# alessioGalatolo/GAN-2D-to-3D

Hardware: AMD Instinct MI355X
Metric: GAN2Shape step iters/sec, faces 128×128 b=8, 1/2/4/8 MI355X (higher is better)
Workload: dtype f32; 1 GPU; face128_n8; image_size=128, gan_size=128, n_proj_samples=8, mfma_operands=f32, prior=ellipsoid, step_mix=7:7:6 (step1:step2:step3, main.py:148 stage 0), images_per_rank=1

## Files before the change

gan-2d-to-3d_amd/csrc/fused_bias_act.hip:

```cpp
#include "g2s_common.h"
#include <hip/hip_fp16.h>

namespace g2s {

enum { MODE_LIN = 0, MODE_ZERO = 1, MODE_LRELU = 2, MODE_LRELU_GRAD = 3 };

__device__ __forceinline__ float act_apply(int mode, float x, float ref, float alpha, float scale) {
    float y;
    switch (mode) {
    case MODE_ZERO: y = 0.0f; break;
    case MODE_LRELU: y = (x > 0.0f) ? x : x * alpha; break;
    case MODE_LRELU_GRAD: y = (ref > 0.0f) ? x : x * alpha; break;
    default: y = x; break;
    }
    return y * scale;
}

template <int MODE, bool BIAS>
__global__ __launch_bounds__(256) void fba_f32_vec4(const float4 *__restrict__ x,
                                                    const float *__restrict__ b,
                                                    const float4 *__restrict__ ref,
                                                    float4 *__restrict__ y, unsigned n4,
                                                    unsigned step_b4, unsigned size_b, float alpha,
                                                    float scale) {
// ... 166 lines not shown
        noise_bias_act_scalar<<<dim3(std::min(cdiv(HW, 256), 64), B * C), 256, 0, st>>>(
            x, noise, noise_w, bias, y, C, HW, alpha, scale);
    }
    return check_launch("g2s_noise_bias_act");
}

namespace g2s {

__global__ __launch_bounds__(256) void add_bias_scale_kernel(const float *a, const float *b, const float *bias,
                                                             float *y, int64_t n, int64_t hw, int C, float scale) {
    const bool vec = (n & 3) == 0 && (hw & 3) == 0 &&
                     ((reinterpret_cast<uintptr_t>(a) | reinterpret_cast<uintptr_t>(y) | reinterpret_cast<uintptr_t>(b)) & 15) == 0;
    const int64_t stride = (int64_t)gridDim.x * blockDim.x * 4;
    for (int64_t i = ((int64_t)blockIdx.x * blockDim.x + threadIdx.x) * 4; i < n; i += stride) {
        if (vec) {
            float4 v = *reinterpret_cast<const float4 *>(a + i);
            if (b) {
                const float4 w = *reinterpret_cast<const float4 *>(b + i);
                v.x += w.x;
                v.y += w.y;
                v.z += w.z;
                v.w += w.w;
            }
            const float bi = bias ? bias[(i / hw) % C] : 0.0f;
            *reinterpret_cast<float4 *>(y + i) = float4{(v.x + bi) * scale, (v.y + bi) * scale, (v.z + bi) * scale,
                                                        (v.w + bi) * scale};
        } else {
            for (int64_t j = i; j < i + 4 && j < n; j++)
                y[j] = (a[j] + (b ? b[j] : 0.0f) + (bias ? bias[(j / hw) % C] : 0.0f)) * scale;
        }
    }
}

__global__ void clamp_kernel(const float *__restrict__ x, const float *__restrict__ g, float *__restrict__ y,
                             int64_t n, float lo, float hi, int dir) {
    const int64_t stride = (int64_t)gridDim.x * blockDim.x * 4;
    for (int64_t i = ((int64_t)blockIdx.x * blockDim.x + threadIdx.x) * 4; i < n; i += stride) {
        if (i + 4 <= n && (((uintptr_t)(x + i) | (uintptr_t)(y + i) | (uintptr_t)(dir ? g + i : x + i)) & 15) == 0) {
            const float4 v = *reinterpret_cast<const float4 *>(x + i);
            float4 o;
            if (dir) {
                const float4 q = *reinterpret_cast<const float4 *>(g + i);
                o = float4{(v.x >= lo && v.x <= hi) ? q.x : 0.0f, (v.y >= lo && v.y <= hi) ? q.y : 0.0f,
                           (v.z >= lo && v.z <= hi) ? q.z : 0.0f, (v.w >= lo && v.w <= hi) ? q.w : 0.0f};
            } else {
                auto cl = [&](float t) { return t < lo ? lo : (t > hi ? hi : t); };
                o = float4{cl(v.x), cl(v.y), cl(v.z), cl(v.w)};
            }
            *reinterpret_cast<float4 *>(y + i) = o;
        } else {
            for (int64_t j = i; j < i + 4 && j < n; j++)
                y[j] = dir ? ((x[j] >= lo && x[j] <= hi) ? g[j] : 0.0f) : (x[j] < lo ? lo : (x[j] > hi ? hi : x[j]));
        }
    }
}

}

extern "C" int g2s_clamp(const float *x, const float *g, float *y, int64_t n, float lo, float hi, int backward,
                         g2s_stream_t stream) {
    G2S_REQUIRE(x && y && n > 0 && (!backward || g) && lo <= hi, "bad argument");
    const int64_t quads = (n + 3) / 4;
    const int blocks = (int)std::min<int64_t>((quads + 255) / 256, 256 * 8);
    g2s::clamp_kernel<<<blocks, 256, 0, g2s::as_stream(stream)>>>(x, g, y, n, lo, hi, backward ? 1 : 0);
    return g2s::check_launch("g2s_clamp");
}

extern "C" int g2s_add_bias_scale(const float *a, const float *b, const float *bias, float *y, int64_t n, int64_t hw,
                                  int C, float scale, g2s_stream_t stream) {
    G2S_REQUIRE(a && y, "a and y must not be NULL");
    G2S_REQUIRE(n > 0 && hw > 0 && C > 0, "n, hw, C must be positive");
    const int64_t quads = (n + 3) / 4;
    const int blocks = (int)std::min<int64_t>((quads + 255) / 256, 256 * 8);
    g2s::add_bias_scale_kernel<<<blocks, 256, 0, g2s::as_stream(stream)>>>(a, b, bias, y, n, hw, C, scale);
    return g2s::check_launch("g2s_add_bias_scale");
}
```

gan-2d-to-3d_amd/csrc/rowops.hip:

```cpp
#include <algorithm>
#include "g2s_common.h"
#include "wave_sum.h"

namespace g2s {

__global__ __launch_bounds__(256) void rows_dot_scale(const float *__restrict__ a,
                                                      const float *__restrict__ b,
                                                      const float *__restrict__ s,
                                                      const float *__restrict__ inv,
                                                      float *__restrict__ out,
                                                      float *__restrict__ dot, int rows, int n,
                                                      int aligned_bases) {
    const int row = blockIdx.x * 4 + (threadIdx.x >> 6), lane = threadIdx.x & 63;
    if (row >= rows) return;
    const size_t off = (size_t)row * n;
    const float *ar = a ? a + off : nullptr;
    const float *br = b + off;
    float *orow = out ? out + off : nullptr;
    const float sc = s ? s[row] : 1.0f;
    float acc = 0.0f;
    int head = aligned_bases ? (int)((4 - (off & 3)) & 3) : n;
    if (head > n) head = n;
    const int n4 = (n - head) >> 2, tail0 = head + 4 * n4;
    for (int i = lane; i < head; i += 64) {
// ... 39 lines not shown
    __shared__ float red[4][64];
    const int lane = threadIdx.x & 63, wave = threadIdx.x >> 6;
    float acc = 0.0f;
    if (i < Cin) {
#pragma unroll 8
        for (int o = wave; o < Cout; o += 4) {
            const float d = demod[b * Cout + o];
            acc += gd[b * Cout + o] * d * d * d * wsq[(size_t)o * Cin + i];
        }
    }
    red[wave][lane] = acc;
    __syncthreads();
    if (wave == 0 && i < Cin) {
        const float g = -s[b * Cin + i] * (red[0][lane] + red[1][lane] + red[2][lane] + red[3][lane]);
        store(b * Cin + i, g);
    }
}

__global__ __launch_bounds__(256) void demod_fwd(const float *__restrict__ wsq, const float *__restrict__ s,
                                                 float *__restrict__ demod, int B, int Cin, int Cout, float eps) {
    const int idx = blockIdx.x * 4 + (threadIdx.x >> 6);
    if (idx >= B * Cout) return;
    demod_fwd_one(wsq, s, demod, idx, threadIdx.x & 63, Cin, Cout, eps);
}

__global__ __launch_bounds__(256) void demod_bwd(const float *__restrict__ wsq, const float *__restrict__ s,
                                                 const float *__restrict__ demod, const float *__restrict__ gd,
                                                 const float *gs_add,
                                                 float *gs, int B, int Cin, int Cout) {
    demod_bwd_one(wsq, s, demod, gd, blockIdx.x * 64 + (threadIdx.x & 63), blockIdx.y, Cin, Cout,
                  [=](int at, float g) { gs[at] = gs_add ? gs_add[at] + g : g; });
}

__global__ __launch_bounds__(256) void synth_rows(const float *__restrict__ x, const float *__restrict__ g1,
                                                  const float *__restrict__ s1, const float *__restrict__ g2,
                                                  const float *__restrict__ s2, const float *__restrict__ noise,
                                                  const float *__restrict__ noise_w, const float *__restrict__ bias,
                                                  const float *__restrict__ demod, float *__restrict__ out,
                                                  float *__restrict__ dot1, float *__restrict__ dot2,
                                                  float *__restrict__ gdot, int rows, int channels, int n,
                                                  int noise_stride, float slope, float gain, int vec) {
    const int row = blockIdx.x * 4 + (threadIdx.x >> 6), lane = threadIdx.x & 63;
    if (row >= rows) return;
    const size_t off = (size_t)row * n;
    const float *xr = x + off, *g1r = g1 + off, *g2r = g2 ? g2 + off : nullptr;
    float *orow = out ? out + off : nullptr;
    const float a1 = s1[row], a2 = g2 ? s2[row] : 0.0f;
    float nw = 0.0f, bi = 0.0f;
    if (gdot) {
        const int b = row / channels;
        nw = noise_w[0];
        bi = bias[row - b * channels];
        noise += (size_t)b * noise_stride;
    }
    const float inv_gain = 1.0f / gain, inv_slope = 1.0f / slope;
    float d1 = 0.0f, d2 = 0.0f, dg = 0.0f;
    auto one = [&](float xv, float gv1, float gv2, float nz) {
        d1 += xv * gv1;
        d2 += xv * gv2;
        const float o = (gv1 * a1 + gv2 * a2) * (xv > 0.0f ? gain : gain * slope);
        if (gdot) dg += o * ((xv > 0.0f ? xv : xv * inv_slope) * inv_gain - nw * nz - bi);
        return o;
    };
    if (vec) {
        for (int i = lane; i < (n >> 2); i += 64) {
            const float4 xv = reinterpret_cast<const float4 *>(xr)[i];
            const float4 v1 = reinterpret_cast<const float4 *>(g1r)[i];
            const float4 v2 = g2r ? reinterpret_cast<const float4 *>(g2r)[i] : float4{0.f, 0.f, 0.f, 0.f};
            const float4 nz = gdot ? reinterpret_cast<const float4 *>(noise)[i] : float4{0.f, 0.f, 0.f, 0.f};
            float4 o;
            o.x = one(xv.x, v1.x, v2.x, nz.x);
            o.y = one(xv.y, v1.y, v2.y, nz.y);
            o.z = one(xv.z, v1.z, v2.z, nz.z);
            o.w = one(xv.w, v1.w, v2.w, nz.w);
            if (orow) reinterpret_cast<float4 *>(orow)[i] = o;
        }
    } else {
        for (int i = lane; i < n; i += 64) {
            const float o = one(xr[i], g1r[i], g2r ? g2r[i] : 0.0f, gdot ? noise[i] : 0.0f);
            if (orow) orow[i] = o;
        }
    }
    d1 = wave_sum(d1);
    d2 = wave_sum(d2);
    dg = wave_sum(dg);
    if (lane == 0) {
        dot1[row] = d1;
        if (dot2) dot2[row] = d2;
        if (gdot) gdot[row] = dg / demod[row];
    }
}

__global__ __launch_bounds__(256) void channel_sum(const float *__restrict__ g, float *__restrict__ out, int B, int C,
                                                   int n) {
    __shared__ float red[4];
    const int c = blockIdx.x, lane = threadIdx.x & 63, wave = threadIdx.x >> 6;
    float acc = 0.0f;
    const int total = B * n;
    for (int i = threadIdx.x; i < total; i += 256) acc += g[((size_t)(i / n) * C + c) * n + i % n];
    acc = wave_sum(acc);
    if (lane == 0) red[wave] = acc;
    __syncthreads();
    if (threadIdx.x == 0) out[c] = red[0] + red[1] + red[2] + red[3];
}

struct DemodMulti {
    const float *wsq[G2S_DEMOD_MAX_LAYERS], *s[G2S_DEMOD_MAX_LAYERS], *gd[G2S_DEMOD_MAX_LAYERS];
    float *demod[G2S_DEMOD_MAX_LAYERS], *gs[G2S_DEMOD_MAX_LAYERS];
    int Cin[G2S_DEMOD_MAX_LAYERS], Cout[G2S_DEMOD_MAX_LAYERS];
    int layers, B;
    float eps;
};

__global__ __launch_bounds__(256) void demod_fwd_multi(DemodMulti d) {
    const int l = blockIdx.y;
    const int idx = blockIdx.x * 4 + (threadIdx.x >> 6);
    if (idx >= d.B * d.Cout[l]) return;
    demod_fwd_one(d.wsq[l], d.s[l], d.demod[l], idx, threadIdx.x & 63, d.Cin[l], d.Cout[l], d.eps);
}

// ... 44 lines not shown

extern "C" int g2s_demod_bwd_multi(const void *const *wsq, const void *const *s, const void *const *demod,
                                   const void *const *gd, const void *const *gs, const int *Cin, const int *Cout,
                                   int layers, int B, g2s_stream_t stream) {
    G2S_REQUIRE(gd && gs, "gd, gs must not be NULL");
    DemodMulti d{};
    int mi, mo;
    const int rc = demod_multi_fill(d, wsq, s, demod, gd, gs, Cin, Cout, layers, B, mi, mo);
    if (rc != G2S_OK) return rc;
    for (int l = 0; l < layers; l++) G2S_REQUIRE(gd[l] && gs[l], "layer %d: gd / gs NULL", l);
    demod_bwd_multi<<<dim3(cdiv(mi, 64), B, layers), 256, 0, as_stream(stream)>>>(d);
    return check_launch("g2s_demod_bwd_multi");
}

extern "C" int g2s_channel_sum(const float *g, float *out, int B, int C, int n, g2s_stream_t stream) {
    G2S_REQUIRE(g && out && B > 0 && C > 0 && n > 0 && (long)B * n < (1l << 31), "bad argument");
    channel_sum<<<C, 256, 0, as_stream(stream)>>>(g, out, B, C, n);
    return check_launch("g2s_channel_sum");
}

static int synth_bwd_rows_launch(const char *who, int noise_stride, const float *x, const float *g1, const float *s1,
                                 const float *g2, const float *s2, const float *noise, const float *noise_w,
                                 const float *bias, const float *demod, float *out, float *dot1, float *dot2,
                                 float *gdot, int rows, int channels, int n, float slope, float gain,
                                 g2s_stream_t stream) {
    G2S_REQUIRE(x && g1 && s1 && dot1 && rows > 0 && channels > 0 && n > 0, "x, g1, s1, dot1 must not be NULL; sizes positive");
    G2S_REQUIRE((g2 == nullptr) == (s2 == nullptr) && (g2 == nullptr) == (dot2 == nullptr), "g2, s2, dot2 come together");
    G2S_REQUIRE(!gdot || (noise && noise_w && bias && demod), "gdot needs noise, noise_w, bias, demod");
    G2S_REQUIRE(slope > 0.0f && gain > 0.0f, "slope and gain must be positive (the activation is inverted)");
    uintptr_t bits = (uintptr_t)x | (uintptr_t)g1 | (uintptr_t)g2 | (uintptr_t)out | (gdot ? (uintptr_t)noise : 0);
    const int vec = (n % 4 == 0) && (bits & 15) == 0;
    if (noise_stride)
        G2S_REQUIRE(rows % channels == 0, "rows must be a multiple of channels with one noise map per sample");
    synth_rows<<<cdiv(rows, 4), 256, 0, as_stream(stream)>>>(x, g1, s1, g2, s2, noise, noise_w, bias, demod, out, dot1,
                                                               dot2, gdot, rows, channels, n, noise_stride, slope, gain,
                                                               vec);
    return check_launch(who);
}

extern "C" int g2s_synth_bwd_rows(const float *x, const float *g1, const float *s1, const float *g2, const float *s2,
                                  const float *noise, const float *noise_w, const float *bias, const float *demod,
                                  float *out, float *dot1, float *dot2, float *gdot, int rows, int channels, int n,
                                  float slope, float gain, g2s_stream_t stream) {
    return synth_bwd_rows_launch("g2s_synth_bwd_rows", 0, x, g1, s1, g2, s2, noise, noise_w, bias, demod, out, dot1,
                                 dot2, gdot, rows, channels, n, slope, gain, stream);
}

extern "C" int g2s_synth_bwd_rows_ps(const float *x, const float *g1, const float *s1, const float *g2, const float *s2,
                                     const float *noise, const float *noise_w, const float *bias, const float *demod,
                                     float *out, float *dot1, float *dot2, float *gdot, int rows, int channels, int n,
                                     float slope, float gain, g2s_stream_t stream) {
    return synth_bwd_rows_launch("g2s_synth_bwd_rows_ps", n, x, g1, s1, g2, s2, noise, noise_w, bias, demod, out, dot1,
                                 dot2, gdot, rows, channels, n, slope, gain, stream);
}

extern "C" int g2s_rows_dot_scale(const float *a, const float *b, const float *s, const float *inv,
                                  float *out, float *dot, int rows, int n, g2s_stream_t stream) {
    G2S_REQUIRE(b != nullptr && rows > 0 && n > 0, "b must not be NULL; rows, n positive");
    G2S_REQUIRE(out || dot, "nothing to compute");
    G2S_REQUIRE(!dot || a, "dot needs a");
    const int aligned = !((uintptr_t)b & 15) && (!a || !((uintptr_t)a & 15)) && (!out || !((uintptr_t)out & 15));
    hipStream_t st = as_stream(stream);
    rows_dot_scale<<<cdiv(rows, 4), 256, 0, st>>>(a, b, s, inv, out, dot, rows, n, aligned);
    return check_launch("g2s_rows_dot_scale");
}

extern "C" int g2s_demod_fwd(const float *wsq, const float *s, float *demod, int B, int Cin, int Cout,
                             float eps, g2s_stream_t stream) {
    G2S_REQUIRE(wsq && s && demod && B > 0 && Cin > 0 && Cout > 0, "bad argument");
    demod_fwd<<<cdiv((long)B * Cout, 4), 256, 0, as_stream(stream)>>>(wsq, s, demod, B, Cin, Cout, eps);
    return check_launch("g2s_demod_fwd");
}

extern "C" int g2s_demod_bwd(const float *wsq, const float *s, const float *demod, const float *gd,
                             float *gs, int B, int Cin, int Cout, g2s_stream_t stream) {
    G2S_REQUIRE(wsq && s && demod && gd && gs && B > 0 && Cin > 0 && Cout > 0, "bad argument");
    demod_bwd<<<dim3(cdiv(Cin, 64), B), 256, 0, as_stream(stream)>>>(wsq, s, demod, gd, nullptr, gs, B, Cin, Cout);
    return check_launch("g2s_demod_bwd");
}

extern "C" int g2s_demod_bwd_add(const float *wsq, const float *s, const float *demod, const float *gd,
                                 const float *gs_add, float *gs, int B, int Cin, int Cout, g2s_stream_t stream) {
    G2S_REQUIRE(wsq && s && demod && gd && gs && B > 0 && Cin > 0 && Cout > 0, "bad argument");
    demod_bwd<<<dim3(cdiv(Cin, 64), B), 256, 0, as_stream(stream)>>>(wsq, s, demod, gd, gs_add, gs, B, Cin, Cout);
    return check_launch("g2s_demod_bwd_add");
}
// ... 1 lines not shown
```

gan-2d-to-3d_amd/lib.py:

```python
import ctypes as C
import os

import torch

_HERE = os.path.dirname(os.path.abspath(__file__))
LIB_PATH = os.path.join(_HERE, "lib", "libg2s.so")

G2S_F32, G2S_F16 = 0, 1
CONV_PLAIN, CONV_UP2, CONV_DOWN2 = 0, 1, 2

_lib = None

_p, _i, _f, _sz, _i64, _d = C.c_void_p, C.c_int, C.c_float, C.c_size_t, C.c_int64, C.c_double
SIGNATURES = {
    "g2s_abi_version": (_i, []),
    "g2s_last_error": (C.c_char_p, []),
    "g2s_clamp": (_i, [_p, _p, _p, _i64, _f, _f, _i, _p]),
    "g2s_avg_pyramid": (_i, [_p, _p, _i, _i64, _i, _i, _p]),
    "g2s_res_split_fwd": (_i, [_p, _p, _p, _i64, _i, _i, _p]),
    "g2s_res_split_bwd": (_i, [_p, _p, _p, _p, _i64, _i, _i, _p]),
    "g2s_depth_head_fwd": (_i, [_p, _p, _p, _i64, _i, _f, _f, _i, _f, _p]),
    "g2s_depth_head_bwd": (_i, [_p, _p, _p, _p, _p, _i64, _i, _f, _f, _i, _f, _i, _p]),
    "g2s_grid_sample_fwd": (_i, [_p, _p, _p, _i, _i, _i, _i, _i, _i, _i, _f, _f, _p]),
    "g2s_grid_sample_bwd_workspace_bytes": (_sz, [_i, _i, _i, _i]),
# ... 5 lines not shown
    "g2s_raster_get_tune": (_i, []),
    "g2s_raster_depth_fwd": (_i, [_p, _p, _i, _i, _i, _i, _p, _f, _i, _i, _f, _f, _p, _p, _p, _p, _sz, _p]),
    "g2s_raster_depth_bwd": (_i, [_p, _p, _p, _p, _p, _i, _i, _i, _i, _p, _f, _i, _p, _p]),
    "g2s_raster_bwd_workspace_bytes": (_sz, [_i, _i]),
    "g2s_raster_depth_bwd_ex": (_i, [_p, _p, _p, _p, _p, _i, _i, _i, _i, _p, _f, _i, _p, _p, _sz, _i, _p]),
    "g2s_raster_rgb_fwd": (_i, [_p, _p, _p, _p, _p, _i, _i, _i, _i, _i, _i, _i, _p, _f, _p, _p]),
    "g2s_raster_rgb_bwd_workspace_bytes": (_sz, [_i, _i, _i, _i, _i]),
    "g2s_raster_rgb_bwd": (_i, [_p] * 6 + [_i, _i, _i, _i, _p, _f, _i, _i, _i, _f, _p, _p, _p, _sz, _i, _p]),
    "g2s_face_light_fwd": (_i, [_p, _p, _i, _i, _i, _i, _i, _p, _p, _p, _p, _p]),
    "g2s_face_light_bwd": (_i, [_p, _p, _p, _i, _i, _i, _i, _i, _p, _p, _p, _p, _sz, _i, _p]),
    "g2s_raster_rgba_fwd": (_i, [_p] * 6 + [_i, _i, _i, _i, _i, _i, _i, _i, _p, _f, _p, _p, _p]),
    "g2s_raster_rgba_bwd_workspace_bytes": (_sz, [_i, _i, _i, _i, _i, _i]),
    "g2s_raster_rgba_bwd": (_i, [_p] * 7 + [_i, _i, _i, _i, _p, _f, _i, _i, _i, _i, _f, _p, _p, _p, _p, _sz, _i, _p]),
    "g2s_sweep_verts": (_i, [_p, _p, _p, _i, _i, _i, _p]),
    "g2s_sweep_shade": (_i, [_p] * 8 + [_i] * 9 + [_p, _f, _p, _p, _p]),
    "g2s_sweep_pseudo": (_i, [_p] * 8 + [_f, _f, _i, _i, _i, _i, _p, _p, _p]),
    "g2s_mapping_tile": (_i, []),
    "g2s_mapping_fwd": (_i, [_p, _p, _p, _p, _p, _p, _i64, _i, _i, _i, _f, _f, _f, _p]),
    "g2s_rows_mean": (_i, [_p, _p, _i64, _i, _i64, _p]),
    "g2s_image_to_u8": (_i, [_p, _p, _i64, _i, _i, _p]),
    "g2s_fused_bias_act": (_i, [_p, _p, _p, _p, _i64, _i64, _i64, _i, _i, _f, _f, _i, _p]),
    "g2s_maxpool2x2_fwd": (_i, [_p, _p, _i64, _i, _i, _p]),
    "g2s_maxpool2x2_bwd": (_i, [_p, _p, _p, _i64, _i, _i, _p]),
    "g2s_add_bias_scale": (_i, [_p, _p, _p, _p, _i64, _i64, _i, _f, _p]),
    "g2s_noise_bias_act": (_i, [_p, _p, _p, _p, _p, _i, _i, _i, _f, _f, _p]),
    "g2s_noise_bias_act_ps": (_i, [_p, _p, _p, _p, _p, _i, _i, _i, _f, _f, _p]),
    "g2s_upfirdn2d": (_i, [_p, _p, _p] + [_i] * 14 + [_p]),
    "g2s_modconv": (_i, [_p] * 8 + [_i] * 9 + [_f, _f, _i, _p]),
    "g2s_modconv_needs_zero": (_i, [_i, _i, _i, _i, _i, _i, _i, _i, _i, _i]),
    "g2s_upfirdn2d_nba": (_i, [_p, _p, _p] + [_i] * 12 + [_p, _p, _p, _f, _f, _p]),
    "g2s_synth_bwd_rows": (_i, [_p] * 13 + [_i, _i, _i, _f, _f, _p]),
    "g2s_upfirdn2d_nba_ps": (_i, [_p, _p, _p] + [_i] * 12 + [_p, _p, _p, _f, _f, _p]),
    "g2s_synth_bwd_rows_ps": (_i, [_p] * 13 + [_i, _i, _i, _f, _f, _p]),
    "g2s_channel_sum": (_i, [_p, _p, _i, _i, _i, _p]),
    "g2s_noise_grad": (_i, [_p, _p, _p, _i, _i, _i, _p]),
    "g2s_noise_regularize_workspace_bytes": (_sz, [_p, _i, _i]),
    "g2s_noise_regularize": (_i, [_p, _p, _p, _i, _i, _p, _p, _sz, _p]),
    "g2s_noise_normalize_workspace_bytes": (_sz, [_p, _i, _i]),
    "g2s_noise_normalize": (_i, [_p, _p, _i, _i, _p, _sz, _p]),
    "g2s_demod_fwd_multi": (_i, [_p, _p, _p, _p, _p, _i, _i, _f, _p]),
    "g2s_demod_bwd_multi": (_i, [_p, _p, _p, _p, _p, _p, _p, _i, _i, _p]),
    "g2s_modconv_f16": (_i, [_p, _p, _p, _p, _p, _p, _i, _i, _i, _i, _i, _i, _i, _i, _i, _f, _f, _p]),
    "g2s_modconv_tune": (_i, [_i, _i]),
    "g2s_mfma_probe": (_i, [_p, _i, _i, _i, _p]),
    "g2s_mfma_lds_probe": (_i, [_p, _i, _i, _i, _i, _p]),
    "g2s_wino_weights_floats": (_sz, [_i, _i]),
    "g2s_wino4_weights_floats": (_sz, [_i, _i]),
    "g2s_wino4_weights": (_i, [_p, _p, _i, _i, _i, _p]),
    "g2s_wino4_supported": (_i, [_i] * 5),
    "g2s_conv3x3_wino4": (_i, [_p] * 8 + [_i] * 6 + [_f, _f, _i, _p, _i64, _p]),
    "g2s_wino_weights": (_i, [_p, _p, _i, _i, _i, _p]),
    "g2s_conv3x3_wino": (_i, [_p] * 8 + [_i] * 6 + [_f, _f, _i, _p, _i64, _p]),
    "g2s_conv2d": (_i, [_p, _p, _p, _p] + [_i] * 12 + [_i, _f, _f, _i, _i, _p]),
    "g2s_conv2d_wgrad": (_i, [_p, _p, _p] + [_i] * 10 + [_i, _i, _p]),
    "g2s_conv2d_bwd": (_i, [_p, _p, _p] + [_i] * 13 + [_p, _p, _p] + [_i] * 8 + [_p]),
    "g2s_adam_chunk": (_i64, []),
    "g2s_adam_step": (_i, [_p, _p, _p, _i, _i, _f, _f, _f, _f, _f, _p]),
    "g2s_rows_dot_scale": (_i, [_p, _p, _p, _p, _p, _p, _i, _i, _p]),
    "g2s_demod_fwd": (_i, [_p, _p, _p, _i, _i, _i, _f, _p]),
    "g2s_demod_bwd": (_i, [_p, _p, _p, _p, _p, _i, _i, _i, _p]),
    "g2s_demod_bwd_add": (_i, [_p, _p, _p, _p, _p, _p, _i, _i, _i, _p]),
    "g2s_lpips_layer_fwd": (_i, [_p, _p, _p, _p, _i, _i, _i, _p]),
    "g2s_lpips_layer_bwd": (_i, [_p, _p, _p, _p, _p, _i, _i, _i, _p]),
    "g2s_lpips_layer_bwd_ex": (_i, [_p, _p, _p, _p, _p, _i, _p, _i, _i, _i, _p]),
    "g2s_weighted_l1_fwd": (_i, [_p, _p, _p, _p, _i, _i, _i, _p]),
    "g2s_weighted_l1_bwd": (_i, [_p, _p, _p, _p, _p, _i, _i, _i, _p]),
# ... 99 lines not shown
```

gan-2d-to-3d_amd/synthesis.py:

```python
import contextlib

import torch
from torch.autograd import Function
from torch.autograd.function import once_differentiable

from . import lib as _lib
from .modconv import PLAIN, UP2, modconv_nba_raw, modconv_raw, rows_dot_scale
from .op.fused_act import add_bias_scale
from .op.upfirdn2d import upfirdn2d, upfirdn2d_adjoint


PER_SAMPLE = False


@contextlib.contextmanager
def per_sample_noise(on=True):
    global PER_SAMPLE
    prev, PER_SAMPLE = PER_SAMPLE, bool(on)
    try:
        yield
    finally:
        PER_SAMPLE = prev


def _ptr_array(tensors):
    return (_lib.C.c_void_p * len(tensors))(*[t.data_ptr() for t in tensors])


def _int_array(values):
    return (_lib.C.c_int * len(values))(*[int(v) for v in values])


def _demod_all(wsqs, styles, eps):
    B = styles[0].shape[0]
    demods = [torch.empty((B, w.shape[0]), dtype=torch.float32, device=w.device) for w in wsqs]
    _lib.check(_lib.load().g2s_demod_fwd_multi(_ptr_array(wsqs), _ptr_array(styles), _ptr_array(demods),
                                               _int_array([w.shape[1] for w in wsqs]), _int_array([w.shape[0] for w in wsqs]),
                                               len(wsqs), B, float(eps), _lib.stream()))
    return demods


def _demod_bwd_all(entries):
    wsqs = [e[0] for e in entries]
    B = entries[0][1].shape[0]
# ... 18 lines not shown
    y = torch.empty((B, C, oh, ow), dtype=torch.float32, device=yc.device)
    L = _lib.load()
    _lib.check((L.g2s_upfirdn2d_nba_ps if ps else L.g2s_upfirdn2d_nba)(_lib.ptr(yc), _lib.ptr(k), _lib.ptr(y), B * C, C, H, W, k.shape[0], k.shape[1],
        1, 1, p0, p1, p0, p1, _lib.ptr(act.bias), _lib.ptr(noise), _lib.ptr(nw),
        float(act.negative_slope), float(act.scale), _lib.stream()))
    return y


def _noise_bias_act_ps_(y, tail):
    B, C, H, W = y.shape
    noise, nw, bias, slope, gain = tail
    _check_map(noise, B, H, W)
    _lib.check(_lib.load().g2s_noise_bias_act_ps(_lib.ptr(y), _lib.ptr(noise), _lib.ptr(nw), _lib.ptr(bias), _lib.ptr(y),
                                                 B, C, H * W, float(slope), float(gain), _lib.stream()))
    return y


def _rows(x, g1, s1, g2=None, s2=None, tail=None, demod=None, want_out=True, ps=False):
    B, C, H, W = x.shape
    noise, nw, bias, slope, gain = tail
    out = torch.empty_like(x) if want_out else None
    dot1 = torch.empty((B, C), dtype=torch.float32, device=x.device)
    dot2 = torch.empty_like(dot1) if g2 is not None else None
    gdot = torch.empty_like(dot1) if demod is not None else None
    L = _lib.load()
    _lib.check((L.g2s_synth_bwd_rows_ps if ps else L.g2s_synth_bwd_rows)(
        _lib.ptr(x), _lib.ptr(g1), _lib.ptr(s1), _lib.ptr(g2), _lib.ptr(s2),
        _lib.ptr(noise if demod is not None else None), _lib.ptr(nw if demod is not None else None),
        _lib.ptr(bias if demod is not None else None), _lib.ptr(demod), _lib.ptr(out), _lib.ptr(dot1), _lib.ptr(dot2),
        _lib.ptr(gdot), B * C, C, H * W, float(slope), float(gain), _lib.stream()))
    return out, dot1, dot2, gdot


def _tail(sc, noise):
    a = sc.activate
    return (noise.contiguous(), sc.noise.weight.detach(), a.bias.detach(), a.negative_slope, a.scale)


def _noise_grad(g_pre, layer):
    B, C, H, W = g_pre.shape
    g = torch.empty((B, 1, H, W), dtype=torch.float32, device=g_pre.device)
    _lib.check(_lib.load().g2s_noise_grad(_lib.ptr(g_pre), _lib.ptr(layer['tail'][1]), _lib.ptr(g), B, C, H * W, _lib.stream()))
    return (g if B == 1 or layer['ps'] else g.sum(0, keepdim=True)).view(layer['noise_shape'])


class _Synthesis(Function):

    @staticmethod
    def forward(ctx, G, noise, x0, *styles):
        ctx.noise_grads = noise is None
        if noise is None:
            styles, noise = styles[:-G.num_layers], styles[-G.num_layers:]
        styles = [s.contiguous() for s in styles]
        layers = []
        rgbs = []
        n = 0
        mods = [m for m, _ in G._style_layers()]
        styled_pos = [i for i, m in enumerate(mods) if m.demodulate]
        weights = {i: mods[i]._weights() for i in styled_pos}
        eps = mods[styled_pos[0]].eps
        assert all(mods[i].eps == eps for i in styled_pos)
        demods = dict(zip(styled_pos, _demod_all([weights[i][1].contiguous() for i in styled_pos],
                                                 [styles[i] for i in styled_pos], eps)))

        def styled(sc, x, nz, up):
            nonlocal n
            s = styles[n]
            (w, wsq), demod = weights[n], demods[n]
            assert mods[n] is sc.conv
            n += 1
            tail = _tail(sc, nz)
            ps = nz.shape[0] != 1
            if up:
                yc = modconv_raw(x, w, s, demod, UP2, 0)
                y = _blur_nba(yc, sc.conv.blur, sc.activate, tail[0], tail[1], ps)
            elif ps:
                yc = None
                y = _noise_bias_act_ps_(modconv_raw(x, w, s, demod, PLAIN, 0), tail)
            else:
                yc = None
                y = modconv_nba_raw(x, w, s, demod, tail[2], tail[0], tail[1], tail[3], tail[4])
            layers.append(dict(up=up, sc=sc, w=w, wsq=wsq.contiguous(), s=s, demod=demod, x=x, yc=yc, y=y, tail=tail,
                               noise_shape=nz.shape, ps=ps))
            return y

        def to_rgb(tr, x, skip):
            nonlocal n
            s = styles[n]
            n += 1
            w, _ = tr.conv._weights()
            rgb = modconv_raw(x, w, s, None, PLAIN, 0)
            rgbs.append(dict(tr=tr, w=w, s=s, up=skip is not None, hw=None if skip is None else tuple(skip.shape[2:])))
            return add_bias_scale(rgb, None if skip is None else tr.upsample(skip), tr.bias.detach())

        out = styled(G.conv1, x0.contiguous(), noise[0], False)
        skip = to_rgb(G.to_rgb1, out, None)
        for conv1, conv2, nz1, nz2, tr in zip(G.convs[::2], G.convs[1::2], noise[1::2], noise[2::2], G.to_rgbs):
            out = styled(conv1, out, nz1, True)
            out = styled(conv2, out, nz2, False)
            skip = to_rgb(tr, out, skip)
        assert n == len(styles)
        ctx.layers, ctx.rgbs = layers, rgbs
        return skip

    @staticmethod
    @once_differentiable
    def backward(ctx, g_img):
        layers, rgbs = ctx.layers, ctx.rgbs
        g_rgb = g_img.contiguous()
        nxt = None
        order = []
        pending = []
        n_styles = 2 + 3 * (len(rgbs) - 1)
        g_noise = {}
        want = [ctx.noise_grads and ctx.needs_input_grad[3 + n_styles + i] for i in range(len(layers))]
        li, ri = len(layers) - 1, len(rgbs) - 1
        while ri >= 0:
            T = rgbs[ri]
            plain = layers[li]
            a = plain['y']
            gxs_rgb = modconv_raw(g_rgb, T['w'], None, None, PLAIN, 1)
            pos_T = 1 if ri == 0 else 1 + 3 * ri
            if nxt is None:
                g_pre, dot_T, _, gdot = _rows(a, gxs_rgb, T['s'], None, None, plain['tail'], plain['demod'],
                                                   ps=plain['ps'])
            else:
                g_pre, dot_U, dot_T, gdot = _rows(a, nxt[0], nxt[1], gxs_rgb, T['s'], plain['tail'], plain['demod'],
                                                       ps=plain['ps'])
                U = nxt[2]
                order.append((nxt[3], dot_U))
                pending.append((U['wsq'], U['s'], U['demod'], U['gd'], dot_U))
            order.append((pos_T, dot_T))
            if want[li]:
                g_noise[li] = _noise_grad(g_pre, plain)
            if T['up']:
                tr = T['tr']
                g_rgb = upfirdn2d_adjoint(g_rgb, tr.upsample.kernel, tr.upsample.factor, 1, tr.upsample.pad, T['hw'])
            gxs_P = modconv_raw(g_pre, plain['w'], plain['demod'], None, PLAIN, 1)
            pos_P = 0 if ri == 0 else 3 * ri
            if ri == 0:
                _, dot_P = rows_dot_scale(plain['x'], gxs_P, None, None, want_out=False, want_dot=True)
                order.append((pos_P, dot_P))
                pending.append((plain['wsq'], plain['s'], plain['demod'], gdot, dot_P))
                break
            up = layers[li - 1]
            g_pre_U, dot_P, _, _ = _rows(up['y'], gxs_P, plain['s'], None, None, up['tail'], None)
            order.append((pos_P, dot_P))
            pending.append((plain['wsq'], plain['s'], plain['demod'], gdot, dot_P))
            if want[li - 1]:
                g_noise[li - 1] = _noise_grad(g_pre_U, up)
            blur = up['sc'].conv.blur
            g_yc = upfirdn2d_adjoint(g_pre_U, blur.kernel, 1, 1, blur.pad, tuple(up['yc'].shape[2:]))
            _, up['gd'] = rows_dot_scale(g_yc, up['yc'], None, up['demod'], want_out=False, want_dot=True)
            gxs_U = modconv_raw(g_yc, up['w'], up['demod'], None, UP2, 1)
            nxt = (gxs_U, up['s'], up, 3 * ri - 1)
            li -= 2
            ri -= 1
        _demod_bwd_all(pending)
        ctx.layers = ctx.rgbs = None
        out = [None] * (max(p for p, _ in order) + 1)
        for p, g in order:
            out[p] = g
        if not ctx.noise_grads:
            return (None, None, None) + tuple(out)
        return (None, None, None) + tuple(out) + tuple(g_noise.get(i) for i in range(len(want)))


def eligible(G, x0, styles, noise):
    from . import modconv as mc
    if mc.OPERANDS != "f32" or not x0.is_cuda or x0.dtype != torch.float32 or any(nz is None for nz in noise):
        return False
    if any(nz.shape[0] != 1 and not (PER_SAMPLE and nz.dim() == 4 and nz.shape[0] == x0.shape[0]) for nz in noise):
        return False
    if any(p.requires_grad for p in G.parameters()):
        return False
    return all(isinstance(s, torch.Tensor) and s.dim() == 2 and s.dtype == torch.float32 for s in styles)


def synthesize(G, noise, x0, styles):
    if torch.is_grad_enabled() and any(nz.requires_grad for nz in noise):
        return _Synthesis.apply(G, None, x0, *styles, *noise)
    return _Synthesis.apply(G, list(noise), x0, *styles)
```

include/g2s.h:

```cpp
#ifndef G2S_H
#define G2S_H

#include <stddef.h>
#include <stdint.h>

#ifdef __cplusplus
extern "C" {
#endif

#define G2S_ABI_VERSION 1

#define G2S_OK 0
#define G2S_ERR_INVALID (-1)
#define G2S_ERR_LAUNCH (-2)
#define G2S_ERR_WORKSPACE (-3)

#define G2S_F32 0
#define G2S_F16 1

typedef void *g2s_stream_t;

int g2s_abi_version(void);
const char *g2s_last_error(void);

// ... 58 lines not shown
                        size_t workspace_bytes, int acc_is_zero, g2s_stream_t stream);

int g2s_sweep_verts(const float *verts, const float *pose, float *out, int B, int V, int n_verts,
                    g2s_stream_t stream);

int g2s_sweep_shade(const float *verts, const int32_t *faces, const int32_t *face_idx, const float *bary,
                    const float *attr, const float *normal, const float *pose, const float *light, int B, int V,
                    int n_verts, int n_faces, int S, int ssaa, int C, int fill_back, int mode,
                    const float *background, float grey, float *rgb_out, float *alpha_out, g2s_stream_t stream);

int g2s_sweep_pseudo(const float *warped, const float *rays, const float *pose, const float *K, const float *albedo,
                     const float *normal, const float *light, const float *mask, float depth_lo, float depth_hi,
                     int B, int V, int S, int C, float *im_out, float *mask_out, g2s_stream_t stream);

int g2s_mapping_tile(void);
int g2s_mapping_fwd(const float *z, const float *w, const float *b, const float *center, float *out,
                    float *partial, int64_t N, int D, int L, int pixel_norm, float alpha, float gain,
                    float truncation, g2s_stream_t stream);

int g2s_rows_mean(const float *partial, float *out, int64_t tiles, int D, int64_t N, g2s_stream_t stream);

int g2s_image_to_u8(const float *x, uint8_t *out, int64_t B, int H, int W, g2s_stream_t stream);

int g2s_fused_bias_act(const void *x, const void *bias, const void *ref, void *y, int64_t n,
                       int64_t step_b, int64_t size_b, int act, int grad, float alpha,
                       float scale, int dtype, g2s_stream_t stream);

int g2s_maxpool2x2_fwd(const float *x, float *y, int64_t planes, int H, int W, g2s_stream_t stream);
int g2s_maxpool2x2_bwd(const float *x, const float *gy, float *gx, int64_t planes, int H, int W,
                       g2s_stream_t stream);

int g2s_add_bias_scale(const float *a, const float *b, const float *bias, float *y, int64_t n, int64_t hw, int C,
                       float scale, g2s_stream_t stream);

int g2s_avg_pyramid(const float *x, float *const *levels, int n_levels, int64_t planes, int H, int W,
                    g2s_stream_t stream);

int g2s_res_split_fwd(const float *x, float *relu_out, float *pool_out, int64_t planes, int H, int W,
                      g2s_stream_t stream);
int g2s_res_split_bwd(const float *x, const float *g_relu, const float *g_pool, float *gx, int64_t planes, int H,
                      int W, g2s_stream_t stream);

int g2s_depth_head_fwd(const float *raw, const float *mean, float *out, int64_t n, int W, float lo, float hi,
                       int clamp_border, float border_depth, g2s_stream_t stream);
int g2s_depth_head_bwd(const float *raw, const float *mean, const float *g, float *g_raw, float *gsum, int64_t n,
                       int W, float lo, float hi, int clamp_border, float border_depth, int acc_is_zero,
                       g2s_stream_t stream);

int g2s_grid_sample_fwd(const float *x, const float *grid, float *y, int B, int C, int IH, int IW, int H, int W,
                        int clamp, float lo, float hi, g2s_stream_t stream);
size_t g2s_grid_sample_bwd_workspace_bytes(int B, int C, int IH, int IW);
int g2s_grid_sample_bwd(const float *gy, const float *x, const float *grid, float *gx, float *ggrid, int B, int C,
                        int IH, int IW, int H, int W, int clamp, float lo, float hi, void *workspace,
                        size_t workspace_bytes, int acc_is_zero, g2s_stream_t stream);

int g2s_clamp(const float *x, const float *g, float *y, int64_t n, float lo, float hi, int backward,
              g2s_stream_t stream);

int g2s_noise_bias_act(const float *x, const float *noise, const float *noise_w,
                       const float *bias, float *y, int B, int C, int HW, float alpha,
                       float scale, g2s_stream_t stream);
int g2s_noise_bias_act_ps(const float *x, const float *noise, const float *noise_w, const float *bias, float *y, int B,
                          int C, int HW, float alpha, float scale, g2s_stream_t stream);

int g2s_upfirdn2d(const void *x, const float *k, void *y, int major, int in_h, int in_w, int kh,
                  int kw, int up_x, int up_y, int down_x, int down_y, int pad_x0, int pad_x1,
// ... 56 lines not shown
int g2s_wino4_supported(int B, int Cr, int M, int H, int W);
int g2s_conv3x3_wino4(const float *x, const float *U, const float *in_scale, const float *out_scale,
                      const float *bias, const float *noise, const float *noise_w, float *y, int B, int Cr, int M,
                      int H, int W, int act, float alpha, float gain, int splitk, float *ws, int64_t ws_floats,
                      g2s_stream_t stream);

int g2s_mfma_probe(float *out, int blocks, int waves, int iters, g2s_stream_t stream);
int g2s_mfma_lds_probe(float *out, int blocks, int waves, int iters, int acc_agpr, g2s_stream_t stream);

int g2s_modconv_tune(int tile, int splitk);

int g2s_rows_dot_scale(const float *a, const float *b, const float *s, const float *inv, float *out,
                       float *dot, int rows, int n, g2s_stream_t stream);
int g2s_demod_fwd(const float *wsq, const float *s, float *demod, int B, int Cin, int Cout,
                  float eps, g2s_stream_t stream);
int g2s_demod_bwd(const float *wsq, const float *s, const float *demod, const float *gd, float *gs,
                  int B, int Cin, int Cout, g2s_stream_t stream);
int g2s_demod_bwd_add(const float *wsq, const float *s, const float *demod, const float *gd, const float *gs_add,
                      float *gs, int B, int Cin, int Cout, g2s_stream_t stream);
int g2s_channel_sum(const float *g, float *out, int B, int C, int n, g2s_stream_t stream);
#define G2S_DEMOD_MAX_LAYERS 24
int g2s_demod_fwd_multi(const void *const *wsq, const void *const *s, const void *const *demod, const int *Cin,
                        const int *Cout, int layers, int B, float eps, g2s_stream_t stream);
int g2s_demod_bwd_multi(const void *const *wsq, const void *const *s, const void *const *demod, const void *const *gd,
                        const void *const *gs, const int *Cin, const int *Cout, int layers, int B, g2s_stream_t stream);
int g2s_synth_bwd_rows(const float *x, const float *g1, const float *s1, const float *g2, const float *s2,
                       const float *noise, const float *noise_w, const float *bias, const float *demod, float *out,
                       float *dot1, float *dot2, float *gdot, int rows, int channels, int n, float slope, float gain,
                       g2s_stream_t stream);
int g2s_synth_bwd_rows_ps(const float *x, const float *g1, const float *s1, const float *g2, const float *s2,
                          const float *noise, const float *noise_w, const float *bias, const float *demod, float *out,
                          float *dot1, float *dot2, float *gdot, int rows, int channels, int n, float slope, float gain,
                          g2s_stream_t stream);

#define G2S_NOISE_MAX_MAPS 32
int g2s_noise_grad(const float *gpre, const float *noise_w, float *gnoise, int B, int C, int n, g2s_stream_t stream);
size_t g2s_noise_regularize_workspace_bytes(const int *sides, int maps, int B);
int g2s_noise_regularize(const void *const *noise, const void *const *grad, const int *sides, int maps, int B,
                         float *loss, void *workspace, size_t workspace_bytes, g2s_stream_t stream);
size_t g2s_noise_normalize_workspace_bytes(const int *sides, int maps, int B);
int g2s_noise_normalize(const void *const *noise, const int *sides, int maps, int B, void *workspace,
                        size_t workspace_bytes, g2s_stream_t stream);

int g2s_lpips_layer_fwd(const float *f0, const float *f1, const float *w, float *out, int N, int C,
                        int HW, g2s_stream_t stream);
int g2s_lpips_layer_bwd(const float *f0, const float *f1, const float *w, const float *gout,
                        float *g0, int N, int C, int HW, g2s_stream_t stream);
int g2s_lpips_layer_bwd_ex(const float *f0, const float *f1, const float *w, const float *gout,
                           const float *g_in, int relu_gate, float *g0, int N, int C, int HW,
                           g2s_stream_t stream);

int g2s_weighted_l1_fwd(const float *x, const float *y, const float *w, float *num, int B, int C, int HW,
                        g2s_stream_t stream);
int g2s_weighted_l1_bwd(const float *x, const float *y, const float *w, const float *coef, float *gx, int B,
                        int C, int HW, g2s_stream_t stream);
int g2s_weighted_l1_fwd2(const float *x, const float *y, const float *w, float *numden, int B, int C, int HW,
                         g2s_stream_t stream);
int g2s_weighted_l1_bwd2(const float *x, const float *y, const float *w, const float *g, const float *den,
                         const float *gadd, float *gx, int B, int C, int HW, g2s_stream_t stream);
int g2s_weighted_l1_bwd3(const float *x, const float *y, const float *w, const float *g, const float *den,
                         const float *gadd, const float *gadd2, float add_scale, float *gx, const float *gate_ref,
                         float slope, float gain, float *gx_gate, int B, int C, int HW, g2s_stream_t stream);


int g2s_view_transform_fwd(const float *view, float rot_scale, float txy_scale, float tz_scale,
                           float *R, float *t, int B, g2s_stream_t stream);
// ... 77 lines not shown
```

Before: 205.9 iters/s.

## Fuse toRGB backward mix into synthesis row kernel and fuse skip upsample join

In the StyleGAN synthesis custom autograd path, the toRGB backward 1x1 modconv (expanding the 3-channel RGB gradient back to C channels) is folded into the row-wise backward kernel, which now reads the three RGB gradient planes and mixes them per channel. The forward skip path gets a fused upfirdn upsample plus add plus bias kernel in place of a separate upsample and add_bias_scale. The upsampled layer's demod gradient now comes from the rows kernel's gdot instead of a separate rows_dot_scale over the stored pre-blur conv output, so that tensor no longer needs to be kept. These changes remove intermediate tensors and kernel launches at the cost of a scalar, non-vectorised gather loop in the join kernel.

```diff
diff --git a/gan-2d-to-3d_amd/csrc/fused_bias_act.hip b/gan-2d-to-3d_amd/csrc/fused_bias_act.hip
--- a/gan-2d-to-3d_amd/csrc/fused_bias_act.hip
+++ b/gan-2d-to-3d_amd/csrc/fused_bias_act.hip
@@ -222,6 +222,30 @@
     }
 }
 
+__global__ __launch_bounds__(256) void rgb_join_kernel(const float *__restrict__ rgb, const float *__restrict__ skip,
+                                                       const float *__restrict__ bias, const float *__restrict__ k,
+                                                       float *__restrict__ out, int64_t total, int channels, int in_h,
+                                                       int in_w, int out_h, int out_w, int kh, int kw, int up, int pad0) {
+    for (int64_t i = (int64_t)blockIdx.x * blockDim.x + threadIdx.x; i < total; i += (int64_t)gridDim.x * blockDim.x) {
+        const int ox = (int)(i % out_w);
+        const int oy = (int)((i / out_w) % out_h);
+        const int64_t m = i / ((int64_t)out_w * out_h);
+        const float *sm = skip + m * in_h * in_w;
+        const int ky0 = ((pad0 - oy) % up + up) % up, kx0 = ((pad0 - ox) % up + up) % up;
+        float acc = 0.0f;
+        for (int ky = ky0; ky < kh; ky += up) {
+            const int uy = oy + ky - pad0;
+            if (uy < 0 || uy / up >= in_h) continue;
+            for (int kx = kx0; kx < kw; kx += up) {
+                const int ux = ox + kx - pad0;
+                if (ux < 0 || ux / up >= in_w) continue;
+                acc += sm[(size_t)(uy / up) * in_w + ux / up] * k[(kh - 1 - ky) * kw + (kw - 1 - kx)];
+            }
+        }
+        out[i] = rgb[i] + acc + bias[m % channels];
+    }
+}
+
 __global__ void clamp_kernel(const float *__restrict__ x, const float *__restrict__ g, float *__restrict__ y,
                              int64_t n, float lo, float hi, int dir) {
     const int64_t stride = (int64_t)gridDim.x * blockDim.x * 4;
@@ -265,3 +289,21 @@
     g2s::add_bias_scale_kernel<<<blocks, 256, 0, g2s::as_stream(stream)>>>(a, b, bias, y, n, hw, C, scale);
     return g2s::check_launch("g2s_add_bias_scale");
 }
+
+extern "C" int g2s_rgb_join(const float *rgb, const float *skip, const float *bias, const float *k, float *out, int planes,
+                            int channels, int in_h, int in_w, int out_h, int out_w, int kh, int kw, int up, int pad0,
+                            int pad1, g2s_stream_t stream) {
+    G2S_REQUIRE(rgb && skip && bias && k && out, "rgb, skip, bias, k, out must not be NULL");
+    G2S_REQUIRE(planes > 0 && channels > 0 && planes % channels == 0 && in_h > 0 && in_w > 0 && kh > 0 && kw > 0 && up > 0,
+                "sizes must be positive; planes a multiple of channels");
+    G2S_REQUIRE(pad0 >= 0 && pad1 >= 0, "pads must not be negative");
+    G2S_REQUIRE(out_h == in_h * up + pad0 + pad1 - kh + 1 && out_w == in_w * up + pad0 + pad1 - kw + 1 && out_h > 0 &&
+                    out_w > 0,
+                "rgb is %d x %d, the up-sampled skip %d x %d", out_h, out_w, in_h * up + pad0 + pad1 - kh + 1,
+                in_w * up + pad0 + pad1 - kw + 1);
+    const int64_t total = (int64_t)planes * out_h * out_w;
+    const int blocks = (int)std::min<int64_t>((total + 255) / 256, 256 * 8);
+    g2s::rgb_join_kernel<<<blocks, 256, 0, g2s::as_stream(stream)>>>(rgb, skip, bias, k, out, total, channels, in_h, in_w,
+                                                                      out_h, out_w, kh, kw, up, pad0);
+    return g2s::check_launch("g2s_rgb_join");
+}
diff --git a/gan-2d-to-3d_amd/csrc/rowops.hip b/gan-2d-to-3d_amd/csrc/rowops.hip
--- a/gan-2d-to-3d_amd/csrc/rowops.hip
+++ b/gan-2d-to-3d_amd/csrc/rowops.hip
@@ -95,6 +95,7 @@
                   [=](int at, float g) { gs[at] = gs_add ? gs_add[at] + g : g; });
 }
 
+template <bool RGB>
 __global__ __launch_bounds__(256) void synth_rows(const float *__restrict__ x, const float *__restrict__ g1,
                                                   const float *__restrict__ s1, const float *__restrict__ g2,
                                                   const float *__restrict__ s2, const float *__restrict__ noise,
@@ -102,13 +103,14 @@
                                                   const float *__restrict__ demod, float *__restrict__ out,
                                                   float *__restrict__ dot1, float *__restrict__ dot2,
                                                   float *__restrict__ gdot, int rows, int channels, int n,
-                                                  int noise_stride, float slope, float gain, int vec) {
+                                                  int noise_stride, float slope, float gain, int vec,
+                                                  const float *__restrict__ w_rgb) {
     const int row = blockIdx.x * 4 + (threadIdx.x >> 6), lane = threadIdx.x & 63;
     if (row >= rows) return;
     const size_t off = (size_t)row * n;
-    const float *xr = x + off, *g1r = g1 + off, *g2r = g2 ? g2 + off : nullptr;
+    const float *xr = x + off, *g1r = (RGB && !g1) ? nullptr : g1 + off, *g2r = (g2 && !RGB) ? g2 + off : nullptr;
     float *orow = out ? out + off : nullptr;
-    const float a1 = s1[row], a2 = g2 ? s2[row] : 0.0f;
+    const float a1 = (RGB && !g1) ? 0.0f : s1[row], a2 = g2 ? s2[row] : 0.0f;
     float nw = 0.0f, bi = 0.0f;
     if (gdot) {
         const int b = row / channels;
@@ -116,6 +118,18 @@
         bi = bias[row - b * channels];
         noise += (size_t)b * noise_stride;
     }
+    const float *r0 = nullptr, *r1 = nullptr, *r2 = nullptr;
+    float w0 = 0.0f, w1 = 0.0f, w2 = 0.0f;
+    if (RGB) {
+        const int b = row / channels, c = row - b * channels;
+        r0 = g2 + (size_t)b * 3 * n;
+        r1 = r0 + n;
+        r2 = r1 + n;
+        w0 = w_rgb[c];
+        w1 = w_rgb[channels + c];
+        w2 = w_rgb[2 * channels + c];
+    }
+    auto mix = [&](float p, float q, float r) { return w0 * p + w1 * q + w2 * r; };
     const float inv_gain = 1.0f / gain, inv_slope = 1.0f / slope;
     float d1 = 0.0f, d2 = 0.0f, dg = 0.0f;
     auto one = [&](float xv, float gv1, float gv2, float nz) {
@@ -128,8 +142,16 @@
     if (vec) {
         for (int i = lane; i < (n >> 2); i += 64) {
             const float4 xv = reinterpret_cast<const float4 *>(xr)[i];
-            const float4 v1 = reinterpret_cast<const float4 *>(g1r)[i];
-            const float4 v2 = g2r ? reinterpret_cast<const float4 *>(g2r)[i] : float4{0.f, 0.f, 0.f, 0.f};
+            const float4 v1 = (RGB && !g1r) ? float4{0.f, 0.f, 0.f, 0.f} : reinterpret_cast<const float4 *>(g1r)[i];
+            float4 v2;
+            if (RGB) {
+                const float4 p = reinterpret_cast<const float4 *>(r0)[i];
+                const float4 q = reinterpret_cast<const float4 *>(r1)[i];
+                const float4 r = reinterpret_cast<const float4 *>(r2)[i];
+                v2 = float4{mix(p.x, q.x, r.x), mix(p.y, q.y, r.y), mix(p.z, q.z, r.z), mix(p.w, q.w, r.w)};
+            } else {
+                v2 = g2r ? reinterpret_cast<const float4 *>(g2r)[i] : float4{0.f, 0.f, 0.f, 0.f};
+            }
             const float4 nz = gdot ? reinterpret_cast<const float4 *>(noise)[i] : float4{0.f, 0.f, 0.f, 0.f};
             float4 o;
             o.x = one(xv.x, v1.x, v2.x, nz.x);
@@ -140,7 +162,9 @@
         }
     } else {
         for (int i = lane; i < n; i += 64) {
-            const float o = one(xr[i], g1r[i], g2r ? g2r[i] : 0.0f, gdot ? noise[i] : 0.0f);
+            const float gv1 = (RGB && !g1r) ? 0.0f : g1r[i];
+            const float gv2 = RGB ? mix(r0[i], r1[i], r2[i]) : (g2r ? g2r[i] : 0.0f);
+            const float o = one(xr[i], gv1, gv2, gdot ? noise[i] : 0.0f);
             if (orow) orow[i] = o;
         }
     }
@@ -148,7 +172,7 @@
     d2 = wave_sum(d2);
     dg = wave_sum(dg);
     if (lane == 0) {
-        dot1[row] = d1;
+        if (!RGB || dot1) dot1[row] = d1;
         if (dot2) dot2[row] = d2;
         if (gdot) gdot[row] = dg / demod[row];
     }
@@ -259,9 +283,9 @@
     const int vec = (n % 4 == 0) && (bits & 15) == 0;
     if (noise_stride)
         G2S_REQUIRE(rows % channels == 0, "rows must be a multiple of channels with one noise map per sample");
-    synth_rows<<<cdiv(rows, 4), 256, 0, as_stream(stream)>>>(x, g1, s1, g2, s2, noise, noise_w, bias, demod, out, dot1,
-                                                               dot2, gdot, rows, channels, n, noise_stride, slope, gain,
-                                                               vec);
+    synth_rows<false><<<cdiv(rows, 4), 256, 0, as_stream(stream)>>>(x, g1, s1, g2, s2, noise, noise_w, bias, demod, out,
+                                                                      dot1, dot2, gdot, rows, channels, n, noise_stride,
+                                                                      slope, gain, vec, nullptr);
     return check_launch(who);
 }
 
@@ -279,6 +303,26 @@
                                      float slope, float gain, g2s_stream_t stream) {
     return synth_bwd_rows_launch("g2s_synth_bwd_rows_ps", n, x, g1, s1, g2, s2, noise, noise_w, bias, demod, out, dot1,
                                  dot2, gdot, rows, channels, n, slope, gain, stream);
+}
+
+extern "C" int g2s_synth_bwd_rows_rgb(const float *x, const float *g1, const float *s1, const float *g_rgb,
+                                      const float *w_rgb, const float *s2, const float *noise, const float *noise_w,
+                                      const float *bias, const float *demod, float *out, float *dot1, float *dot2,
+                                      float *gdot, int rows, int channels, int n, int noise_stride, float slope,
+                                      float gain, g2s_stream_t stream) {
+    G2S_REQUIRE(x && g_rgb && w_rgb && s2 && dot2 && rows > 0 && channels > 0 && n > 0,
+                "x, g_rgb, w_rgb, s2, dot2 must not be NULL; sizes positive");
+    G2S_REQUIRE((g1 == nullptr) == (s1 == nullptr) && (g1 == nullptr) == (dot1 == nullptr), "g1, s1, dot1 come together");
+    G2S_REQUIRE(rows % channels == 0, "rows must be a multiple of channels (row r reads g_rgb of sample r / channels)");
+    G2S_REQUIRE(noise_stride == 0 || noise_stride == n, "noise_stride is 0 (one map) or n (one map per sample)");
+    G2S_REQUIRE(!gdot || (noise && noise_w && bias && demod), "gdot needs noise, noise_w, bias, demod");
+    G2S_REQUIRE(slope > 0.0f && gain > 0.0f, "slope and gain must be positive (the activation is inverted)");
+    uintptr_t bits = (uintptr_t)x | (uintptr_t)g1 | (uintptr_t)g_rgb | (uintptr_t)out | (gdot ? (uintptr_t)noise : 0);
+    const int vec = (n % 4 == 0) && (bits & 15) == 0;
+    synth_rows<true><<<cdiv(rows, 4), 256, 0, as_stream(stream)>>>(x, g1, s1, g_rgb, s2, noise, noise_w, bias, demod, out,
+                                                                     dot1, dot2, gdot, rows, channels, n, noise_stride,
+                                                                     slope, gain, vec, w_rgb);
+    return check_launch("g2s_synth_bwd_rows_rgb");
 }
 
 extern "C" int g2s_rows_dot_scale(const float *a, const float *b, const float *s, const float *inv,
diff --git a/gan-2d-to-3d_amd/lib.py b/gan-2d-to-3d_amd/lib.py
--- a/gan-2d-to-3d_amd/lib.py
+++ b/gan-2d-to-3d_amd/lib.py
@@ -61,6 +61,8 @@
     "g2s_synth_bwd_rows": (_i, [_p] * 13 + [_i, _i, _i, _f, _f, _p]),
     "g2s_upfirdn2d_nba_ps": (_i, [_p, _p, _p] + [_i] * 12 + [_p, _p, _p, _f, _f, _p]),
     "g2s_synth_bwd_rows_ps": (_i, [_p] * 13 + [_i, _i, _i, _f, _f, _p]),
+    "g2s_synth_bwd_rows_rgb": (_i, [_p] * 14 + [_i, _i, _i, _i, _f, _f, _p]),
+    "g2s_rgb_join": (_i, [_p] * 5 + [_i] * 11 + [_p]),
     "g2s_channel_sum": (_i, [_p, _p, _i, _i, _i, _p]),
     "g2s_noise_grad": (_i, [_p, _p, _p, _i, _i, _i, _p]),
     "g2s_noise_regularize_workspace_bytes": (_sz, [_p, _i, _i]),
diff --git a/gan-2d-to-3d_amd/synthesis.py b/gan-2d-to-3d_amd/synthesis.py
--- a/gan-2d-to-3d_amd/synthesis.py
+++ b/gan-2d-to-3d_amd/synthesis.py
@@ -10,6 +10,7 @@
 from .op.upfirdn2d import upfirdn2d, upfirdn2d_adjoint
 
 
+FUSED_RGB = True
 PER_SAMPLE = False
 
 
@@ -94,6 +95,35 @@
     return out, dot1, dot2, gdot
 
 
+def _rows_rgb(x, g1, s1, g_rgb, w_rgb, s2, tail, demod, ps=False):
+    B, C, H, W = x.shape
+    noise, nw, bias, slope, gain = tail
+    if tuple(g_rgb.shape) != (B, 3, H, W) or tuple(w_rgb.shape) != (3, C, 1, 1):
+        raise RuntimeError(f"synthesis: g_rgb {tuple(g_rgb.shape)} / w_rgb {tuple(w_rgb.shape)} do not fit x {tuple(x.shape)}")
+    g_rgb, w_rgb = g_rgb.contiguous(), w_rgb.contiguous()
+    out = torch.empty_like(x)
+    dot1 = torch.empty((B, C), dtype=torch.float32, device=x.device) if g1 is not None else None
+    dot2 = torch.empty((B, C), dtype=torch.float32, device=x.device)
+    gdot = torch.empty_like(dot2)
+    _lib.check(_lib.load().g2s_synth_bwd_rows_rgb(
+        _lib.ptr(x), _lib.ptr(g1), _lib.ptr(s1), _lib.ptr(g_rgb), _lib.ptr(w_rgb), _lib.ptr(s2), _lib.ptr(noise),
+        _lib.ptr(nw), _lib.ptr(bias), _lib.ptr(demod), _lib.ptr(out), _lib.ptr(dot1), _lib.ptr(dot2), _lib.ptr(gdot), B * C, C,
+        H * W, H * W if ps else 0, float(slope), float(gain), _lib.stream()))
+    return out, dot1, dot2, gdot
+
+
+def _rgb_join(rgb, skip, bias, up):
+    B, C, H, W = rgb.shape
+    k, skip, bias = up.kernel.contiguous(), skip.contiguous(), bias.reshape(-1).contiguous()
+    if k.dtype != torch.float32 or tuple(skip.shape[:2]) != (B, C) or bias.numel() != C:
+        raise RuntimeError(f"synthesis: skip {tuple(skip.shape)} / bias {tuple(bias.shape)} do not fit rgb {tuple(rgb.shape)}")
+    out = torch.empty_like(rgb)
+    _lib.check(_lib.load().g2s_rgb_join(_lib.ptr(rgb), _lib.ptr(skip), _lib.ptr(bias),
+                                        _lib.ptr(k), _lib.ptr(out), B * C, C, skip.shape[2], skip.shape[3], H, W,
+                                        k.shape[0], k.shape[1], int(up.factor), int(up.pad[0]), int(up.pad[1]), _lib.stream()))
+    return out
+
+
 def _tail(sc, noise):
     a = sc.activate
     return (noise.contiguous(), sc.noise.weight.detach(), a.bias.detach(), a.negative_slope, a.scale)
@@ -114,6 +144,7 @@
         if noise is None:
             styles, noise = styles[:-G.num_layers], styles[-G.num_layers:]
         styles = [s.contiguous() for s in styles]
+        fused_rgb = ctx.fused_rgb = FUSED_RGB
         layers = []
         rgbs = []
         n = 0
@@ -133,17 +164,17 @@
             n += 1
             tail = _tail(sc, nz)
             ps = nz.shape[0] != 1
+            yc_hw = None
             if up:
                 yc = modconv_raw(x, w, s, demod, UP2, 0)
+                yc_hw = tuple(yc.shape[2:])
                 y = _blur_nba(yc, sc.conv.blur, sc.activate, tail[0], tail[1], ps)
             elif ps:
-                yc = None
                 y = _noise_bias_act_ps_(modconv_raw(x, w, s, demod, PLAIN, 0), tail)
             else:
-                yc = None
                 y = modconv_nba_raw(x, w, s, demod, tail[2], tail[0], tail[1], tail[3], tail[4])
-            layers.append(dict(up=up, sc=sc, w=w, wsq=wsq.contiguous(), s=s, demod=demod, x=x, yc=yc, y=y, tail=tail,
-                               noise_shape=nz.shape, ps=ps))
+            layers.append(dict(up=up, sc=sc, w=w, wsq=wsq.contiguous(), s=s, demod=demod, x=x, y=y, tail=tail,
+                               noise_shape=nz.shape, ps=ps, yc_hw=yc_hw))
             return y
 
         def to_rgb(tr, x, skip):
@@ -153,6 +184,8 @@
             w, _ = tr.conv._weights()
             rgb = modconv_raw(x, w, s, None, PLAIN, 0)
             rgbs.append(dict(tr=tr, w=w, s=s, up=skip is not None, hw=None if skip is None else tuple(skip.shape[2:])))
+            if skip is not None and fused_rgb:
+                return _rgb_join(rgb, skip, tr.bias.detach(), tr.upsample)
             return add_bias_scale(rgb, None if skip is None else tr.upsample(skip), tr.bias.detach())
 
         out = styled(G.conv1, x0.contiguous(), noise[0], False)
@@ -181,14 +214,19 @@
             T = rgbs[ri]
             plain = layers[li]
             a = plain['y']
-            gxs_rgb = modconv_raw(g_rgb, T['w'], None, None, PLAIN, 1)
             pos_T = 1 if ri == 0 else 1 + 3 * ri
-            if nxt is None:
-                g_pre, dot_T, _, gdot = _rows(a, gxs_rgb, T['s'], None, None, plain['tail'], plain['demod'],
-                                                   ps=plain['ps'])
+            if ctx.fused_rgb:
+                g_pre, dot_U, dot_T, gdot = _rows_rgb(a, None if nxt is None else nxt[0], None if nxt is None else nxt[1],
+                                                      g_rgb, T['w'], T['s'], plain['tail'], plain['demod'], ps=plain['ps'])
             else:
-                g_pre, dot_U, dot_T, gdot = _rows(a, nxt[0], nxt[1], gxs_rgb, T['s'], plain['tail'], plain['demod'],
-                                                       ps=plain['ps'])
+                gxs_rgb = modconv_raw(g_rgb, T['w'], None, None, PLAIN, 1)
+                if nxt is None:
+                    g_pre, dot_T, _, gdot = _rows(a, gxs_rgb, T['s'], None, None, plain['tail'], plain['demod'],
+                                                  ps=plain['ps'])
+                else:
+                    g_pre, dot_U, dot_T, gdot = _rows(a, nxt[0], nxt[1], gxs_rgb, T['s'], plain['tail'], plain['demod'],
+                                                      ps=plain['ps'])
+            if nxt is not None:
                 U = nxt[2]
                 order.append((nxt[3], dot_U))
                 pending.append((U['wsq'], U['s'], U['demod'], U['gd'], dot_U))
@@ -206,14 +244,14 @@
                 pending.append((plain['wsq'], plain['s'], plain['demod'], gdot, dot_P))
                 break
             up = layers[li - 1]
-            g_pre_U, dot_P, _, _ = _rows(up['y'], gxs_P, plain['s'], None, None, up['tail'], None)
+            g_pre_U, dot_P, _, up['gd'] = _rows(up['y'], gxs_P, plain['s'], None, None, up['tail'], up['demod'],
+                                                ps=up['ps'])
             order.append((pos_P, dot_P))
             pending.append((plain['wsq'], plain['s'], plain['demod'], gdot, dot_P))
             if want[li - 1]:
                 g_noise[li - 1] = _noise_grad(g_pre_U, up)
             blur = up['sc'].conv.blur
-            g_yc = upfirdn2d_adjoint(g_pre_U, blur.kernel, 1, 1, blur.pad, tuple(up['yc'].shape[2:]))
-            _, up['gd'] = rows_dot_scale(g_yc, up['yc'], None, up['demod'], want_out=False, want_dot=True)
+            g_yc = upfirdn2d_adjoint(g_pre_U, blur.kernel, 1, 1, blur.pad, up['yc_hw'])
             gxs_U = modconv_raw(g_yc, up['w'], up['demod'], None, UP2, 1)
             nxt = (gxs_U, up['s'], up, 3 * ri - 1)
             li -= 2
diff --git a/include/g2s.h b/include/g2s.h
--- a/include/g2s.h
+++ b/include/g2s.h
@@ -114,6 +114,9 @@
 
 int g2s_add_bias_scale(const float *a, const float *b, const float *bias, float *y, int64_t n, int64_t hw, int C,
                        float scale, g2s_stream_t stream);
+int g2s_rgb_join(const float *rgb, const float *skip, const float *bias, const float *k, float *out, int planes,
+                 int channels, int in_h, int in_w, int out_h, int out_w, int kh, int kw, int up, int pad0, int pad1,
+                 g2s_stream_t stream);
 
 int g2s_avg_pyramid(const float *x, float *const *levels, int n_levels, int64_t planes, int H, int W,
                     g2s_stream_t stream);
@@ -236,6 +239,10 @@
                           const float *noise, const float *noise_w, const float *bias, const float *demod, float *out,
                           float *dot1, float *dot2, float *gdot, int rows, int channels, int n, float slope, float gain,
                           g2s_stream_t stream);
+int g2s_synth_bwd_rows_rgb(const float *x, const float *g1, const float *s1, const float *g_rgb, const float *w_rgb,
+                           const float *s2, const float *noise, const float *noise_w, const float *bias,
+                           const float *demod, float *out, float *dot1, float *dot2, float *gdot, int rows, int channels,
+                           int n, int noise_stride, float slope, float gain, g2s_stream_t stream);
 
 #define G2S_NOISE_MAX_MAPS 32
 int g2s_noise_grad(const float *gpre, const float *noise_w, float *gnoise, int B, int C, int n, g2s_stream_t stream);
```

Result: no change. 204.4 iters/s (-0.7%).
